# psy-ex/svt-av1-psy

Measured on AMD Instinct MI355X. Metric: Mblocks/s per kernel (SAD, FwdTxfm2d, CDEF) + encoder fps @1080p preset 8, higher is better.
Workload: dtype u8

## Files before the change

svt-av1-psy_amd/csrc/cdef_pick.hip:

```cpp
#include "svt_hip_common.h"
#include "../../include/svtav1_hip.h"

#include <vector>

namespace {

constexpr int NS = 64;

__global__ __launch_bounds__(256) void search_best_kernel(const unsigned long long* __restrict__ mse0, const unsigned long long* __restrict__ mse1,
                                                          const int* __restrict__ lev0, const int* __restrict__ lev1, const int nb_strengths, const int sb_count,
                                                          unsigned long long* __restrict__ best, unsigned long long* __restrict__ tot) {
    const int i = blockIdx.x * blockDim.x + threadIdx.x;
    if (i < NS * NS) tot[i] = 0;
    if (i >= sb_count) return;
    unsigned long long b = 1ull << 63;
    for (int gi = 0; gi < nb_strengths; gi++) {
        const unsigned long long c = mse0[(size_t)i * NS + lev0[gi]] + mse1[(size_t)i * NS + lev1[gi]];
        b = c < b ? c : b;
    }
    best[i] = b;
}
constexpr int SLICE = 128;
__global__ __launch_bounds__(256) void search_tot_kernel(const unsigned long long* __restrict__ mse0, const unsigned long long* __restrict__ mse1,
                                                         const unsigned long long* __restrict__ best, const int sb_count, const int start_gi,
                                                         unsigned long long* __restrict__ tot) {
    __shared__ unsigned long long part[4][NS];
    const int j = start_gi + blockIdx.x, k = threadIdx.x & 63, sl = threadIdx.x >> 6;
    const int i0 = blockIdx.y * SLICE, i1 = i0 + SLICE < sb_count ? i0 + SLICE : sb_count;
    unsigned long long acc = 0;
    for (int i = i0 + sl; i < i1; i += 4) {
        const unsigned long long c = mse0[(size_t)i * NS + j] + mse1[(size_t)i * NS + k], b = best[i];
        acc += c < b ? c : b;
    }
    part[sl][k] = acc;
    __syncthreads();
    if (sl == 0) atomicAdd(&tot[j * NS + k], part[0][k] + part[1][k] + part[2][k] + part[3][k]);
}
__global__ __launch_bounds__(256) void search_pick_kernel(const unsigned long long* __restrict__ tot, const int start_gi, const int end_gi, int* __restrict__ lev0,
                                                          int* __restrict__ lev1, const int nb_strengths, unsigned long long* __restrict__ out_best) {
    __shared__ unsigned long long wv_tot[4];
    __shared__ int                wv_arg[4];
    const int tid = threadIdx.x;
    unsigned long long t = ~0ull;
    int                a = NS * NS;
    for (int e = tid; e < NS * NS; e += 256) {
        const int j = e >> 6, k = e & 63;
        if (j >= start_gi && j < end_gi && k >= start_gi && k < end_gi) {
            const unsigned long long v = tot[e];
            if (v < t || (v == t && e < a)) { t = v; a = e; }
        }
    }
#pragma unroll
    for (int m = 32; m >= 1; m >>= 1) {
        const unsigned long long t2 = (unsigned long long)__shfl_xor((long long)t, m);
        const int                a2 = __shfl_xor(a, m);
        if (t2 < t || (t2 == t && a2 < a)) { t = t2; a = a2; }
    }
    if ((tid & 63) == 0) { wv_tot[tid >> 6] = t; wv_arg[tid >> 6] = a; }
    __syncthreads();
    if (tid == 0) {
        for (int w = 1; w < 4; w++)
            if (wv_tot[w] < t || (wv_tot[w] == t && wv_arg[w] < a)) { t = wv_tot[w]; a = wv_arg[w]; }
        const bool won = a < NS * NS && t < (1ull << 63);
        lev0[nb_strengths] = won ? a >> 6 : 0;
        lev1[nb_strengths] = won ? a & 63 : 0;
        out_best[0]        = won ? t : (1ull << 63);
    }
}

__global__ void shift_levels_kernel(int* lev0, int* lev1, const int nb_strengths) {
    if (threadIdx.x == 0 && blockIdx.x == 0)
        for (int j = 0; j < nb_strengths - 1; j++) { lev0[j] = lev0[j + 1]; lev1[j] = lev1[j + 1]; }
}
__global__ __launch_bounds__(256) void assign_fb_kernel(const unsigned long long* __restrict__ mse0, const unsigned long long* __restrict__ mse1,
                                                        const int* __restrict__ lev0, const int* __restrict__ lev1, const int nb_strengths, const int sb_count,
                                                        int8_t* __restrict__ best_gi) {
    const int i = blockIdx.x * blockDim.x + threadIdx.x;
    if (i >= sb_count) return;
    unsigned long long best = 1ull << 63;
    int                arg  = 0;
    for (int gi = 0; gi < nb_strengths; gi++) {
        const unsigned long long c = mse0[(size_t)i * NS + lev0[gi]] + mse1[(size_t)i * NS + lev1[gi]];
        if (c < best) { best = c; arg = gi; }
    }
    best_gi[i] = (int8_t)arg;
}

}

extern "C" {

void svt_hip_cdef_search_one_dual(const uint64_t* mse0, const uint64_t* mse1, int* lev0, int* lev1, int nb_strengths, int sb_count, int start_gi,
                                  int end_gi, uint64_t* best_tot_mse, void* workspace, void* stream) {
    svthip::ensure_device();
    hipStream_t st = (hipStream_t)stream;
    unsigned long long* tot  = (unsigned long long*)workspace;
    unsigned long long* best = tot + NS * NS;
    const int nrows = end_gi - start_gi, cover = sb_count > NS * NS ? sb_count : NS * NS;
    hipLaunchKernelGGL(search_best_kernel, dim3((cover + 255) / 256), dim3(256), 0, st, (const unsigned long long*)mse0, (const unsigned long long*)mse1,
                       (const int*)lev0, (const int*)lev1, nb_strengths, sb_count, best, tot);
    SVT_LAUNCH_CHECK();
    if (nrows > 0 && sb_count > 0) {
        hipLaunchKernelGGL(search_tot_kernel, dim3(nrows, (sb_count + SLICE - 1) / SLICE), dim3(256), 0, st, (const unsigned long long*)mse0,
                           (const unsigned long long*)mse1, (const unsigned long long*)best, sb_count, start_gi, tot);
        SVT_LAUNCH_CHECK();
    }
    hipLaunchKernelGGL(search_pick_kernel, dim3(1), dim3(256), 0, st, (const unsigned long long*)tot, start_gi, end_gi, lev0, lev1, nb_strengths,
                       (unsigned long long*)best_tot_mse);
    SVT_LAUNCH_CHECK();
}

void svt_hip_cdef_joint_strength_search(const uint64_t* mse0, const uint64_t* mse1, int* lev0, int* lev1, int nb_strengths, int sb_count, int start_gi,
                                        int end_gi, uint64_t* best_tot_mse, void* workspace, void* stream) {
    for (int i = 0; i < nb_strengths; i++)
        svt_hip_cdef_search_one_dual(mse0, mse1, lev0, lev1, i, sb_count, start_gi, end_gi, best_tot_mse, workspace, stream);
    for (int i = 0; i < 4 * nb_strengths; i++) {
        hipLaunchKernelGGL(shift_levels_kernel, dim3(1), dim3(64), 0, (hipStream_t)stream, lev0, lev1, nb_strengths);
        SVT_LAUNCH_CHECK();
        svt_hip_cdef_search_one_dual(mse0, mse1, lev0, lev1, nb_strengths - 1, sb_count, start_gi, end_gi, best_tot_mse, workspace, stream);
    }
}

void svt_hip_cdef_assign_fb_strengths(const uint64_t* mse0, const uint64_t* mse1, const int* lev0, const int* lev1, int nb_strengths, int sb_count,
                                      int8_t* best_gi, void* stream) {
    svthip::ensure_device();
    if (sb_count <= 0) return;
    hipLaunchKernelGGL(assign_fb_kernel, dim3((sb_count + 255) / 256), dim3(256), 0, (hipStream_t)stream, (const unsigned long long*)mse0,
                       (const unsigned long long*)mse1, lev0, lev1, nb_strengths, sb_count, best_gi);
    SVT_LAUNCH_CHECK();
}

uint64_t svt_search_one_dual_hip(int* lev0, int* lev1, int nb_strengths, uint64_t** mse[2], int sb_count, int start_gi, int end_gi) {
    svthip::HostCall& c = svthip::host_call();
    c.begin();
    const size_t tbl = (size_t)sb_count * NS * 8;
    c.reserve(2 * tbl + (size_t)(NS * NS + sb_count + 1) * 8 + 8192, 2 * tbl + 8192);
    uint64_t* d0 = (uint64_t*)c.dalloc(tbl ? tbl : 8);
    uint64_t* d1 = (uint64_t*)c.dalloc(tbl ? tbl : 8);
    int*      dl0 = (int*)c.dalloc((NS + 1) * 4);
    int*      dl1 = (int*)c.dalloc((NS + 1) * 4);
    uint64_t* dbest = (uint64_t*)c.dalloc(8);
    void*     ws = c.dalloc((size_t)(NS * NS + sb_count + 1) * 8);
    std::vector<uint64_t> h((size_t)sb_count * NS + 1);
    for (int p = 0; p < 2; p++) {
        for (int i = 0; i < sb_count; i++) memcpy(h.data() + (size_t)i * NS, mse[p][i], NS * 8);
        if (tbl) c.up(p ? d1 : d0, h.data(), tbl);
    }
    c.up(dl0, lev0, nb_strengths * 4);
    c.up(dl1, lev1, nb_strengths * 4);
    svt_hip_cdef_search_one_dual(d0, d1, dl0, dl1, nb_strengths, sb_count, start_gi, end_gi, dbest, ws, c.stream);
    uint64_t best;
    int      a, b;
    c.down_later(&best, dbest, 8);
    c.down_later(&a, dl0 + nb_strengths, 4);
    c.down_later(&b, dl1 + nb_strengths, 4);
    c.finish();
    lev0[nb_strengths] = a;
    lev1[nb_strengths] = b;
    return best;
}

}

SVT_HIP_DEFINE_WARM(cdef_pick)
```

Before: 23490.

## Tile CDEF joint strength search into 4x4 pair tiles with ring-buffered level history

Replaces the three-kernel best/totals/pick pipeline with a tiled kernel where each block computes a 4x4 tile of (j,k) strength-pair totals over all superblocks, reducing in shared memory and emitting a per-tile argmin. The atomicAdd-based totals and the full 64x64 pick scan go away. The joint search loop now keeps the chosen levels in a ring buffer on device and fuses the per-superblock best-cost update into the pick kernel, which removes the shift_levels launches and the per-round best kernel. This means fewer launches and better reuse of the loaded mse rows. The cost is large shared-memory use (16x512 u64 partials per block), which lowers occupancy, plus more complex indexing.

```diff
diff --git a/svt-av1-psy_amd/csrc/cdef_pick.hip b/svt-av1-psy_amd/csrc/cdef_pick.hip
--- a/svt-av1-psy_amd/csrc/cdef_pick.hip
+++ b/svt-av1-psy_amd/csrc/cdef_pick.hip
@@ -6,72 +6,135 @@
 namespace {
 
 constexpr int NS = 64;
-
-__global__ __launch_bounds__(256) void search_best_kernel(const unsigned long long* __restrict__ mse0, const unsigned long long* __restrict__ mse1,
-                                                          const int* __restrict__ lev0, const int* __restrict__ lev1, const int nb_strengths, const int sb_count,
-                                                          unsigned long long* __restrict__ best, unsigned long long* __restrict__ tot) {
-    const int i = blockIdx.x * blockDim.x + threadIdx.x;
-    if (i < NS * NS) tot[i] = 0;
-    if (i >= sb_count) return;
-    unsigned long long b = 1ull << 63;
-    for (int gi = 0; gi < nb_strengths; gi++) {
-        const unsigned long long c = mse0[(size_t)i * NS + lev0[gi]] + mse1[(size_t)i * NS + lev1[gi]];
-        b = c < b ? c : b;
-    }
-    best[i] = b;
-}
-constexpr int SLICE = 128;
-__global__ __launch_bounds__(256) void search_tot_kernel(const unsigned long long* __restrict__ mse0, const unsigned long long* __restrict__ mse1,
-                                                         const unsigned long long* __restrict__ best, const int sb_count, const int start_gi,
-                                                         unsigned long long* __restrict__ tot) {
-    __shared__ unsigned long long part[4][NS];
-    const int j = start_gi + blockIdx.x, k = threadIdx.x & 63, sl = threadIdx.x >> 6;
-    const int i0 = blockIdx.y * SLICE, i1 = i0 + SLICE < sb_count ? i0 + SLICE : sb_count;
-    unsigned long long acc = 0;
-    for (int i = i0 + sl; i < i1; i += 4) {
-        const unsigned long long c = mse0[(size_t)i * NS + j] + mse1[(size_t)i * NS + k], b = best[i];
-        acc += c < b ? c : b;
-    }
-    part[sl][k] = acc;
-    __syncthreads();
-    if (sl == 0) atomicAdd(&tot[j * NS + k], part[0][k] + part[1][k] + part[2][k] + part[3][k]);
-}
-__global__ __launch_bounds__(256) void search_pick_kernel(const unsigned long long* __restrict__ tot, const int start_gi, const int end_gi, int* __restrict__ lev0,
-                                                          int* __restrict__ lev1, const int nb_strengths, unsigned long long* __restrict__ out_best) {
-    __shared__ unsigned long long wv_tot[4];
-    __shared__ int                wv_arg[4];
-    const int tid = threadIdx.x;
-    unsigned long long t = ~0ull;
-    int                a = NS * NS;
-    for (int e = tid; e < NS * NS; e += 256) {
-        const int j = e >> 6, k = e & 63;
-        if (j >= start_gi && j < end_gi && k >= start_gi && k < end_gi) {
-            const unsigned long long v = tot[e];
-            if (v < t || (v == t && e < a)) { t = v; a = e; }
-        }
-    }
+constexpr int TILE = 4, NTILE = NS / TILE;
+constexpr int TT = 512;
+constexpr int SLOTS = 0, RING = 2 * NTILE * NTILE, BEST = NS * NS;
+constexpr unsigned long long NONE = ~0ull;
+
+__device__ __forceinline__ bool smaller(unsigned long long t2, int a2, unsigned long long t, int a) { return t2 < t || (t2 == t && a2 < a); }
+
+__device__ __forceinline__ void wave_min(unsigned long long& t, int& a) {
 #pragma unroll
     for (int m = 32; m >= 1; m >>= 1) {
         const unsigned long long t2 = (unsigned long long)__shfl_xor((long long)t, m);
         const int                a2 = __shfl_xor(a, m);
-        if (t2 < t || (t2 == t && a2 < a)) { t = t2; a = a2; }
-    }
+        if (smaller(t2, a2, t, a)) { t = t2; a = a2; }
+    }
+}
+
+template <bool FROM_LEVELS>
+__global__ __launch_bounds__(TT) void tile_totals_kernel(const unsigned long long* __restrict__ mse0, const unsigned long long* __restrict__ mse1,
+                                                          const unsigned long long* __restrict__ best, const int* __restrict__ lev0, const int* __restrict__ lev1,
+                                                          const int nb_strengths, const int sb_count, const int start_gi, const int end_gi,
+                                                          unsigned long long* __restrict__ slots) {
+    __shared__ unsigned long long part[TILE * TILE][TT];
+    __shared__ unsigned long long wv_tot[TT / 64];
+    __shared__ int                wv_arg[TT / 64];
+    const int tid = threadIdx.x, j0 = blockIdx.x / NTILE * TILE, k0 = blockIdx.x % NTILE * TILE;
+    const int lo = start_gi > 0 ? start_gi : 0, hi = end_gi < NS ? end_gi : NS;
+    if (j0 + TILE <= lo || j0 >= hi || k0 + TILE <= lo || k0 >= hi) {
+        if (tid == 0) { slots[2 * blockIdx.x] = NONE; slots[2 * blockIdx.x + 1] = NS * NS; }
+        return;
+    }
+    unsigned long long acc[TILE * TILE] = {};
+#pragma unroll 2
+    for (int i = tid; i < sb_count; i += TT) {
+        const unsigned long long* r0 = mse0 + (size_t)i * NS + j0;
+        const unsigned long long* r1 = mse1 + (size_t)i * NS + k0;
+        unsigned long long        m0[TILE], m1[TILE];
+#pragma unroll
+        for (int q = 0; q < TILE; q++) { m0[q] = r0[q]; m1[q] = r1[q]; }
+        unsigned long long b = 1ull << 63;
+        if (FROM_LEVELS) {
+            for (int gi = 0; gi < nb_strengths; gi++) {
+                const unsigned long long c = mse0[(size_t)i * NS + lev0[gi]] + mse1[(size_t)i * NS + lev1[gi]];
+                b = c < b ? c : b;
+            }
+        } else {
+            b = best[i];
+        }
+#pragma unroll
+        for (int jj = 0; jj < TILE; jj++)
+#pragma unroll
+            for (int kk = 0; kk < TILE; kk++) {
+                const unsigned long long c = m0[jj] + m1[kk];
+                acc[jj * TILE + kk] += c < b ? c : b;
+            }
+    }
+#pragma unroll
+    for (int c = 0; c < TILE * TILE; c++) part[c][tid] = acc[c];
+    __syncthreads();
+    constexpr int PER = TT / (TILE * TILE);
+    const int     c = tid / PER, q = tid % PER;
+    unsigned long long s = 0;
+#pragma unroll
+    for (int r = 0; r < TT / PER; r++) s += part[c][q + PER * r];
+#pragma unroll
+    for (int m = PER / 2; m >= 1; m >>= 1) s += (unsigned long long)__shfl_xor((long long)s, m);
+    const int          j = j0 + (c >> 2), k = k0 + (c & 3);
+    const bool         in = j >= lo && j < hi && k >= lo && k < hi;
+    unsigned long long t = in ? s : NONE;
+    int                a = in ? j * NS + k : NS * NS;
+    wave_min(t, a);
     if ((tid & 63) == 0) { wv_tot[tid >> 6] = t; wv_arg[tid >> 6] = a; }
     __syncthreads();
     if (tid == 0) {
-        for (int w = 1; w < 4; w++)
-            if (wv_tot[w] < t || (wv_tot[w] == t && wv_arg[w] < a)) { t = wv_tot[w]; a = wv_arg[w]; }
-        const bool won = a < NS * NS && t < (1ull << 63);
-        lev0[nb_strengths] = won ? a >> 6 : 0;
-        lev1[nb_strengths] = won ? a & 63 : 0;
-        out_best[0]        = won ? t : (1ull << 63);
-    }
-}
-
-__global__ void shift_levels_kernel(int* lev0, int* lev1, const int nb_strengths) {
-    if (threadIdx.x == 0 && blockIdx.x == 0)
-        for (int j = 0; j < nb_strengths - 1; j++) { lev0[j] = lev0[j + 1]; lev1[j] = lev1[j + 1]; }
-}
+        for (int w = 1; w < TT / 64; w++)
+            if (smaller(wv_tot[w], wv_arg[w], t, a)) { t = wv_tot[w]; a = wv_arg[w]; }
+        slots[2 * blockIdx.x]     = t;
+        slots[2 * blockIdx.x + 1] = (unsigned long long)a;
+    }
+}
+
+__global__ __launch_bounds__(256) void pick_kernel(const unsigned long long* __restrict__ slots, int* __restrict__ ring, const int ring_n, const int n, const int lo,
+                                                   const unsigned long long* __restrict__ mse0, const unsigned long long* __restrict__ mse1, const int sb_count,
+                                                   unsigned long long* __restrict__ best, int* __restrict__ lev0, int* __restrict__ lev1,
+                                                   unsigned long long* __restrict__ out_best) {
+    __shared__ unsigned long long wv_tot[4];
+    __shared__ int                wv_arg[4];
+    HIP_DYNAMIC_SHARED(int, win)
+    const int tid = threadIdx.x;
+    for (int x = lo + tid; x < n; x += 256) {
+        win[2 * (x - lo)]     = ring[2 * (x % ring_n)];
+        win[2 * (x - lo) + 1] = ring[2 * (x % ring_n) + 1];
+    }
+    unsigned long long t = slots[2 * tid];
+    int                a   = (int)slots[2 * tid + 1];
+    wave_min(t, a);
+    if ((tid & 63) == 0) { wv_tot[tid >> 6] = t; wv_arg[tid >> 6] = a; }
+    __syncthreads();
+    t = wv_tot[0];
+    a = wv_arg[0];
+    for (int w = 1; w < 4; w++)
+        if (smaller(wv_tot[w], wv_arg[w], t, a)) { t = wv_tot[w]; a = wv_arg[w]; }
+    const bool won = t < (1ull << 63);
+    const int  w0 = won ? a >> 6 : 0, w1 = won ? a & (NS - 1) : 0;
+    if (blockIdx.x == 0 && tid == 0) {
+        if (lev0) {
+            for (int x = lo; x <= n; x++) {
+                lev0[x - lo] = x == n ? w0 : win[2 * (x - lo)];
+                lev1[x - lo] = x == n ? w1 : win[2 * (x - lo) + 1];
+            }
+            out_best[0] = won ? t : (1ull << 63);
+        } else {
+            ring[2 * (n % ring_n)]     = w0;
+            ring[2 * (n % ring_n) + 1] = w1;
+        }
+    }
+    const int i = blockIdx.x * blockDim.x + tid;
+    if (lev0 || i >= sb_count) return;
+    const unsigned long long* r0 = mse0 + (size_t)i * NS;
+    const unsigned long long* r1 = mse1 + (size_t)i * NS;
+    unsigned long long        b  = lo <= n ? r0[w0] + r1[w1] : 1ull << 63;
+    b = b < (1ull << 63) ? b : (1ull << 63);
+#pragma unroll 4
+    for (int x = lo; x < n; x++) {
+        const unsigned long long c = r0[win[2 * (x - lo)]] + r1[win[2 * (x - lo) + 1]];
+        b = c < b ? c : b;
+    }
+    best[i] = b;
+}
+
 __global__ __launch_bounds__(256) void assign_fb_kernel(const unsigned long long* __restrict__ mse0, const unsigned long long* __restrict__ mse1,
                                                         const int* __restrict__ lev0, const int* __restrict__ lev1, const int nb_strengths, const int sb_count,
                                                         int8_t* __restrict__ best_gi) {
@@ -93,32 +156,41 @@
 void svt_hip_cdef_search_one_dual(const uint64_t* mse0, const uint64_t* mse1, int* lev0, int* lev1, int nb_strengths, int sb_count, int start_gi,
                                   int end_gi, uint64_t* best_tot_mse, void* workspace, void* stream) {
     svthip::ensure_device();
-    hipStream_t st = (hipStream_t)stream;
-    unsigned long long* tot  = (unsigned long long*)workspace;
-    unsigned long long* best = tot + NS * NS;
-    const int nrows = end_gi - start_gi, cover = sb_count > NS * NS ? sb_count : NS * NS;
-    hipLaunchKernelGGL(search_best_kernel, dim3((cover + 255) / 256), dim3(256), 0, st, (const unsigned long long*)mse0, (const unsigned long long*)mse1,
-                       (const int*)lev0, (const int*)lev1, nb_strengths, sb_count, best, tot);
-    SVT_LAUNCH_CHECK();
-    if (nrows > 0 && sb_count > 0) {
-        hipLaunchKernelGGL(search_tot_kernel, dim3(nrows, (sb_count + SLICE - 1) / SLICE), dim3(256), 0, st, (const unsigned long long*)mse0,
-                           (const unsigned long long*)mse1, (const unsigned long long*)best, sb_count, start_gi, tot);
-        SVT_LAUNCH_CHECK();
-    }
-    hipLaunchKernelGGL(search_pick_kernel, dim3(1), dim3(256), 0, st, (const unsigned long long*)tot, start_gi, end_gi, lev0, lev1, nb_strengths,
-                       (unsigned long long*)best_tot_mse);
+    hipStream_t         st = (hipStream_t)stream;
+    unsigned long long* ws = (unsigned long long*)workspace;
+    hipLaunchKernelGGL(tile_totals_kernel<true>, dim3(NTILE * NTILE), dim3(TT), 0, st, (const unsigned long long*)mse0, (const unsigned long long*)mse1,
+                       (const unsigned long long*)nullptr, (const int*)lev0, (const int*)lev1, nb_strengths, sb_count, start_gi, end_gi, ws + SLOTS);
+    SVT_LAUNCH_CHECK();
+    hipLaunchKernelGGL(pick_kernel, dim3(1), dim3(256), 0, st, (const unsigned long long*)(ws + SLOTS), (int*)nullptr, 1, 0, 0,
+                       (const unsigned long long*)mse0, (const unsigned long long*)mse1, sb_count, (unsigned long long*)nullptr, lev0 + nb_strengths,
+                       lev1 + nb_strengths, (unsigned long long*)best_tot_mse);
     SVT_LAUNCH_CHECK();
 }
 
 void svt_hip_cdef_joint_strength_search(const uint64_t* mse0, const uint64_t* mse1, int* lev0, int* lev1, int nb_strengths, int sb_count, int start_gi,
                                         int end_gi, uint64_t* best_tot_mse, void* workspace, void* stream) {
-    for (int i = 0; i < nb_strengths; i++)
-        svt_hip_cdef_search_one_dual(mse0, mse1, lev0, lev1, i, sb_count, start_gi, end_gi, best_tot_mse, workspace, stream);
-    for (int i = 0; i < 4 * nb_strengths; i++) {
-        hipLaunchKernelGGL(shift_levels_kernel, dim3(1), dim3(64), 0, (hipStream_t)stream, lev0, lev1, nb_strengths);
+    if (nb_strengths <= 0) return;
+    svthip::ensure_device();
+    hipStream_t               st = (hipStream_t)stream;
+    unsigned long long*       ws = (unsigned long long*)workspace;
+    const unsigned long long *m0 = (const unsigned long long*)mse0, *m1 = (const unsigned long long*)mse1;
+    int*                      ring   = (int*)(ws + RING);
+    const int                 rounds = 5 * nb_strengths, nfb_blocks = sb_count > 0 ? (sb_count + 255) / 256 : 1;
+    hipLaunchKernelGGL(tile_totals_kernel<true>, dim3(NTILE * NTILE), dim3(TT), 0, st, m0, m1, (const unsigned long long*)nullptr, (const int*)lev0,
+                       (const int*)lev1, 0, sb_count, start_gi, end_gi, ws + SLOTS);
+    SVT_LAUNCH_CHECK();
+    for (int x = 0; x + 1 < rounds; x++) {
+        const int next = x + 1, lo = next < nb_strengths ? 0 : next - nb_strengths + 1;
+        hipLaunchKernelGGL(pick_kernel, dim3(nfb_blocks), dim3(256), (x > lo ? x - lo : 0) * 8, st, (const unsigned long long*)(ws + SLOTS), ring, nb_strengths, x, lo, m0, m1,
+                           sb_count, ws + BEST, (int*)nullptr, (int*)nullptr, (unsigned long long*)nullptr);
         SVT_LAUNCH_CHECK();
-        svt_hip_cdef_search_one_dual(mse0, mse1, lev0, lev1, nb_strengths - 1, sb_count, start_gi, end_gi, best_tot_mse, workspace, stream);
-    }
+        hipLaunchKernelGGL(tile_totals_kernel<false>, dim3(NTILE * NTILE), dim3(TT), 0, st, m0, m1, (const unsigned long long*)(ws + BEST),
+                           (const int*)nullptr, (const int*)nullptr, 0, sb_count, start_gi, end_gi, ws + SLOTS);
+        SVT_LAUNCH_CHECK();
+    }
+    hipLaunchKernelGGL(pick_kernel, dim3(1), dim3(256), (nb_strengths - 1) * 8, st, (const unsigned long long*)(ws + SLOTS), ring, nb_strengths, rounds - 1,
+                       rounds - nb_strengths, m0, m1, sb_count, (unsigned long long*)nullptr, lev0, lev1, (unsigned long long*)best_tot_mse);
+    SVT_LAUNCH_CHECK();
 }
 
 void svt_hip_cdef_assign_fb_strengths(const uint64_t* mse0, const uint64_t* mse1, const int* lev0, const int* lev1, int nb_strengths, int sb_count,
```

After: 23490, median of 3. No clear change (-0.0%).
